# alexfreudenberg/miraculix

Measured on AMD Instinct MI355X. Metric: effective GFLOP/s for dgemm_compressed (2-bit SNP x fp64), higher is better.
Workload: dtype f64; 1 GPU; 1000000x50000 (SNPs x indiv), ncol=32, dgemm_compressed N+T per step, uncentred; snps=1000000, indiv=50000, ncol=32, parallelism=snp-shard1, form=one process per GPU

## Files before the change

miraculix_amd/csrc/mxa_kernels.hip:

```cpp
#include "mxa_internal.h"
#include "mxa_queue.h"
#include <algorithm>
#include <cstdio>
#include <cstdlib>
#include <vector>

namespace mxa {

constexpr long kMaxBlocksPerLaunch = 1L << 23;

__device__ __forceinline__ uint32_t recode16(uint32_t w) {
  const uint32_t H = (w >> 1) & 0x55555555u, L = w & 0x55555555u;
  return ((H & L) << 1) | (H & ~L);
}

__global__ void __launch_bounds__(256) k_recode(const uint8_t *__restrict__ src, size_t src_pitch, long src_row_bytes,
                                                long nrows, long k, uint8_t *__restrict__ dst, long dst_row0, long nslabs, long rows_blocks, long blk0) {
  const long bid = blk0 + blockIdx.x;
  const long rblk = bid % rows_blocks, sgrp = bid / rows_blocks;
  const int rr = threadIdx.x >> 3, part = threadIdx.x & 7;
  const long r = rblk * 32 + rr;
  const long slab = sgrp * 4 + (part >> 1);
  if (r >= nrows || slab >= nslabs) return;
  const long b = slab * kSlabBytes + (part & 1) * 16;
  uint32_t w[4] = {0u, 0u, 0u, 0u};
  const uint8_t *p = src + (size_t)r * src_pitch + b;
  if (b + 16 <= src_row_bytes && (reinterpret_cast<size_t>(p) & 3) == 0) {
    const uint32_t *q = reinterpret_cast<const uint32_t *>(p);
    w[0] = q[0]; w[1] = q[1]; w[2] = q[2]; w[3] = q[3];
  } else {
    for (int u = 0; u < 16; u++)
      if (b + u < src_row_bytes) w[u >> 2] |= (uint32_t)p[u] << (8 * (u & 3));
  }
#pragma unroll
  for (int i = 0; i < 4; i++) {
    uint32_t x = recode16(w[i]);
    const long valid = k - 4 * (b + 4 * i);
    if (valid <= 0) x = 0;
    else if (valid < 16) x &= (1u << (2 * valid)) - 1u;
    w[i] = x;
  }
  const long R = dst_row0 + r;
  const size_t off = ((size_t)(R / kTileRows) * nslabs + (size_t)slab) * kTileBytes + (size_t)(R % kTileRows) * kSlabBytes + (part & 1) * 16;
  *reinterpret_cast<uint4 *>(dst + off) = make_uint4(w[0], w[1], w[2], w[3]);
}

int launch_recode(const uint8_t *d_src, size_t src_pitch, long row0, long nrows, long k, long ,
                  PackedMatrix &dst, hipStream_t s) {
  if (nrows <= 0) return 0;
  const long rows_blocks = (nrows + 31) / 32, slab_groups = (dst.nslabs + 3) / 4;
  const long grid = rows_blocks * slab_groups;
  for (long b0 = 0; b0 < grid; b0 += kMaxBlocksPerLaunch) {
    const long nb = std::min(kMaxBlocksPerLaunch, grid - b0);
    hipLaunchKernelGGL(k_recode, dim3((unsigned)nb), dim3(256), 0, s, d_src, src_pitch, (k + 3) / 4, nrows, k, dst.d, row0, dst.nslabs, rows_blocks, b0);
  }
  MXA_HIP(hipGetLastError());
  return 0;
}

__host__ __device__ __forceinline__ long gemm_k_index(long S, int kk) { return (S >> 3) * 128 + 16 * (kk & 7) + 8 * (kk >> 3) + (S & 7); }

__global__ void __launch_bounds__(256) k_pack_B(const double *__restrict__ B, long ldb, long k, int n,
                                                double *__restrict__ Bp, long total, int C, long S_total, const int *__restrict__ E, int up, long S0, long S_cnt,
                                                const int *__restrict__ run_if_set, int rowscale) {
  if (run_if_set && *run_if_set == 0) return;
  for (long idx = (long)blockIdx.x * blockDim.x + threadIdx.x; idx < total; idx += (long)gridDim.x * blockDim.x) {
    const int l = (int)(idx & 63);
    const long sh = idx >> 6;
    const int h = (int)(sh % C);
    const long cs = sh / C;
    const long S = S0 + cs % S_cnt;
    const int chunk = (int)(cs / S_cnt);
    const long row = gemm_k_index(S, l >> 2);
    const int col = chunk * 4 * C + 4 * h + (l & 3);
    double v = 0.0;
    if (row < k && col < n) {
      v = B[row + (long)col * ldb];
      if (E) v = ldexp(v, up - E[col] - (rowscale ? 2 * (int)(row & 15) : 0));
    }
    Bp[(((size_t)chunk * S_total + S) * C + h) * 64 + l] = v;
  }
}

__global__ void __launch_bounds__(256) k_colmax_partial(const double *__restrict__ B, long ldb, long k, double *__restrict__ part, int n, int want_min) {
  const int j = blockIdx.y, c = blockIdx.x;
  const long per = (k + 63) / 64;
  const long c0 = c * per, c1 = std::min<long>(k, c0 + per);
  const double inf = __longlong_as_double(0x7ff0000000000000ll);
  double m = 0.0, lo = inf;
  for (long r = c0 + threadIdx.x; r < c1; r += 256) {
    const double a = fabs(B[r + (long)j * ldb]);
    m = (a <= 1.7976931348623157e308) ? fmax(m, a) : inf;
    if (a > 0.0) lo = fmin(lo, a);
  }
  __shared__ double sh[256], sl[256];
  sh[threadIdx.x] = m; sl[threadIdx.x] = lo;
  __syncthreads();
  for (int w = 128; w > 0; w >>= 1) {
    if ((int)threadIdx.x < w) { sh[threadIdx.x] = fmax(sh[threadIdx.x], sh[threadIdx.x + w]); sl[threadIdx.x] = fmin(sl[threadIdx.x], sl[threadIdx.x + w]); }
    __syncthreads();
  }
  if (threadIdx.x == 0) { part[(size_t)j * 64 + c] = sh[0]; if (want_min) part[((size_t)n + j) * 64 + c] = sl[0]; }
}
__global__ void k_colexp_final(const double *__restrict__ part, int n, int bias, int *__restrict__ E, int *__restrict__ flag, int max_span, int min_emax) {
  const int j = blockIdx.x * blockDim.x + threadIdx.x;
  if (j >= n) return;
  double m = 0.0;
  for (int c = 0; c < 64; c++) m = fmax(m, part[(size_t)j * 64 + c]);
  int e = 0;
  if (m > 0.0 && isfinite(m)) (void)frexp(m, &e);
  E[j] = e + bias;
  if (flag) {
    bool ok = isfinite(m);
    if (ok && m > 0.0) {
      double lo = m;
      for (int c = 0; c < 64; c++) lo = fmin(lo, part[((size_t)n + j) * 64 + c]);
      int el = 0;
      (void)frexp(lo, &el);
      ok = e >= min_emax && el >= e - max_span;
    }
    if (!ok) atomicOr(flag, 1);
  }
}
int launch_colexp(const double *dB, long ldb, long k, int n, double *d_part, int *d_E, int bias, hipStream_t s, int *d_flag, int max_span, int min_emax, bool reset_flag) {
  if (d_flag && reset_flag) MXA_HIP(hipMemsetAsync(d_flag, 0, sizeof(int), s));
  hipLaunchKernelGGL(k_colmax_partial, dim3(64, n), dim3(256), 0, s, dB, ldb, k, d_part, n, d_flag ? 1 : 0);
  hipLaunchKernelGGL(k_colexp_final, dim3((n + 63) / 64), dim3(64), 0, s, d_part, n, bias, d_E, d_flag, max_span, min_emax);
  MXA_HIP(hipGetLastError());
  return 0;
}

int launch_colexp_from_part(const double *d_part, int n, int *d_E, int bias, hipStream_t s) {
  hipLaunchKernelGGL(k_colexp_final, dim3((n + 63) / 64), dim3(64), 0, s, d_part, n, bias, d_E, (int *)nullptr, 0, 0);
  MXA_HIP(hipGetLastError());
  return 0;
}

__global__ void __launch_bounds__(256) k_colspan_final(const double *__restrict__ part, int n, int *__restrict__ out) {
  __shared__ int s_span[256], s_emax[256], s_bad[256];
  int span = 0, emin_max = 1 << 20, bad = 0;
  for (int j = threadIdx.x; j < n; j += 256) {
    double m = 0.0;
    for (int c = 0; c < 64; c++) m = fmax(m, part[(size_t)j * 64 + c]);
    if (!isfinite(m)) { bad = 1; continue; }
    if (m > 0.0) {
      double lo = m;
      for (int c = 0; c < 64; c++) lo = fmin(lo, part[((size_t)n + j) * 64 + c]);
      int e = 0, el = 0;
      (void)frexp(m, &e); (void)frexp(lo, &el);
      span = max(span, e - el); emin_max = min(emin_max, e);
    }
  }
  s_span[threadIdx.x] = span; s_emax[threadIdx.x] = emin_max; s_bad[threadIdx.x] = bad;
  __syncthreads();
  for (int w = 128; w > 0; w >>= 1) {
    if ((int)threadIdx.x < w) {
      s_span[threadIdx.x] = max(s_span[threadIdx.x], s_span[threadIdx.x + w]); s_emax[threadIdx.x] = min(s_emax[threadIdx.x], s_emax[threadIdx.x + w]);
      s_bad[threadIdx.x] |= s_bad[threadIdx.x + w];
    }
    __syncthreads();
  }
  if (threadIdx.x == 0) { out[0] = s_span[0]; out[1] = s_emax[0] == (1 << 20) ? 0 : s_emax[0]; out[2] = s_bad[0]; }
}
int launch_colspan(const double *dB, long ldb, long k, int n, double *d_part, int *d_out3, hipStream_t s) {
  hipLaunchKernelGGL(k_colmax_partial, dim3(64, n), dim3(256), 0, s, dB, ldb, k, d_part, n, 1);
  hipLaunchKernelGGL(k_colspan_final, dim3(1), dim3(256), 0, s, d_part, n, d_out3);
  MXA_HIP(hipGetLastError());
  return 0;
}

int launch_pack_B(const double *dB, long ldb, long k, int n, double *dBp, long k_pad, int n_pad, int c, hipStream_t s, const int *d_E, long S0, long S_cnt,
                  const int *run_if_set, bool rowscale) {
  const long S_total = k_pad / 16;
  if (S_cnt < 0) S_cnt = S_total - S0;
  const long total = S_cnt * (long)(n_pad / 4) * 64;
  if (total <= 0) return 0;
  const int grid = (int)std::min<long>((total + 255) / 256, 256L * 64);
  hipLaunchKernelGGL(k_pack_B, dim3(grid), dim3(256), 0, s, dB, ldb, k, n, dBp, total, c, S_total, d_E, kDenUp, S0, S_cnt, run_if_set, rowscale ? 1 : 0);
  MXA_HIP(hipGetLastError());
  return 0;
}

constexpr int kColChunks = 64;

__global__ void __launch_bounds__(256) k_colsum_partial(const double *__restrict__ B, long ldb, long k,
                                                        const double *__restrict__ f, double *__restrict__ part) {
  const int j = blockIdx.y, c = blockIdx.x;
  const long per = (k + kColChunks - 1) / kColChunks;
  const long c0 = c * per, c1 = std::min<long>(k, c0 + per);
  double s1 = 0.0, s2 = 0.0;
  for (long r = c0 + threadIdx.x; r < c1; r += 256) {
    const double b = B[r + (long)j * ldb];
    s1 += b;
    if (f) s2 = fma(f[r], b, s2);
  }
  __shared__ double sh1[256], sh2[256];
  sh1[threadIdx.x] = s1; sh2[threadIdx.x] = s2;
  __syncthreads();
  for (int w = 128; w > 0; w >>= 1) {
    if ((int)threadIdx.x < w) { sh1[threadIdx.x] += sh1[threadIdx.x + w]; sh2[threadIdx.x] += sh2[threadIdx.x + w]; }
    __syncthreads();
  }
  if (threadIdx.x == 0) {
    part[((size_t)j * kColChunks + c) * 2 + 0] = sh1[0];
    part[((size_t)j * kColChunks + c) * 2 + 1] = sh2[0];
  }
}

__global__ void k_colsum_final(const double *__restrict__ part, int n, double *__restrict__ sumB, double *__restrict__ sumfB) {
  const int j = blockIdx.x * blockDim.x + threadIdx.x;
  if (j >= n) return;
  double s1 = 0.0, s2 = 0.0;
  for (int c = 0; c < kColChunks; c++) { s1 += part[((size_t)j * kColChunks + c) * 2]; s2 += part[((size_t)j * kColChunks + c) * 2 + 1]; }
  sumB[j] = s1; sumfB[j] = s2;
}

int launch_colsums(const double *dB, long ldb, long k, int n, const double *d_f, double *d_part, double *d_sumB,
                   double *d_sumfB, hipStream_t s) {
  hipLaunchKernelGGL(k_colsum_partial, dim3(kColChunks, n), dim3(256), 0, s, dB, ldb, k, d_f, d_part);
  hipLaunchKernelGGL(k_colsum_final, dim3((n + 63) / 64), dim3(64), 0, s, d_part, n, d_sumB, d_sumfB);
  MXA_HIP(hipGetLastError());
  return 0;
}

using gptr_t = const __attribute__((address_space(1))) void *;
using lptr_t = __attribute__((address_space(3))) void *;

__device__ __forceinline__ void dma16_s(const void *sbase, uint32_t voff, uint32_t lds_addr) {
  asm volatile("s_mov_b32 m0, %2\n\ts_nop 0\n\tglobal_load_lds_dwordx4 %1, %0" ::"s"(sbase), "v"(voff), "s"(lds_addr) : "memory", "m0");
}
#ifndef MXA_NT_LUT
#define MXA_NT_LUT 0
#endif
#ifndef MXA_NT_GEMM
#define MXA_NT_GEMM 1
#endif
template <bool NT>
__device__ __forceinline__ void dma16_p(const void *sbase, uint32_t voff, uint32_t lds_addr) {
  if (NT) asm volatile("s_mov_b32 m0, %2\n\ts_nop 0\n\tglobal_load_lds_dwordx4 %1, %0 nt" ::"s"(sbase), "v"(voff), "s"(lds_addr) : "memory", "m0");
  else dma16_s(sbase, voff, lds_addr);
}

template <int A, int C>
struct GemmCfg {
  static constexpr int kRowsWave = 4 * A;
  static constexpr int kRowsWG = kWaves * kRowsWave;
  static constexpr int kBBytes = kSlabSteps * C * 512;
  static constexpr int kABytes = kRowsWG * kSlabBytes;
  static constexpr int kBufBytes = kBBytes + kABytes;
  static constexpr int kLds = 2 * kBufBytes;
  static constexpr int kBUnits = kBBytes / 1024;
  static constexpr int kAUnits = kABytes / 1024;
  static_assert(kABytes % 1024 == 0, "A tile must be a whole number of DMA units");
};

template <int A, int C, int MODE, bool DIAG = false, bool TR = false>
__global__ void __launch_bounds__(256, 2)
k_gemm(const uint8_t *__restrict__ G, size_t pitch, const double *__restrict__ Bp, int H, double *__restrict__ P,
       long m_pad, int n_pad, int rowblocks, int nchunks, int slabs_total, KSplit ks, int xcd_order,
       unsigned long long *__restrict__ diag, int split0, const int *__restrict__ run_if_set, int nunits, int *__restrict__ ctr, int g8, int p_split0) {
  using Cfg = GemmCfg<A, C>;
  extern __shared__ __attribute__((aligned(16))) char smem[];
  __shared__ int s_next;
  if (MODE == 0) { if (run_if_set && *run_if_set == 0) return; }

  const int lane = threadIdx.x & 63;
  const int wave = __builtin_amdgcn_readfirstlane(threadIdx.x >> 6);
  PieceQueue q;
  q.init(ctr, rowblocks, g8, nunits);
  auto fetch = [&]() -> int { return q.next(); };

  const uint32_t b_lane = lane * 16;
  const uint32_t a_lane = lane * 16;
  const uint32_t tr_voff = (uint32_t)((16 * ((lane >> 1) & 7) + 8 * ((lane >> 4) & 1) + (lane >> 5)) * kSlabBytes + (lane & 1) * 16);
  const size_t nslabs_all = pitch / kSlabBytes;
  const uint32_t lds0 = (uint32_t)(size_t)(lptr_t)smem;
  struct Unit { int rb, nc, sp, slab0, slab1; const char *Bp_u, *G_u; };
  auto decode = [&](int bid) -> Unit {
    Unit u;
    int grp;
    q.locate(bid, u.rb, grp);
    u.nc = grp % nchunks;
    u.sp = grp / nchunks + split0;
    u.slab0 = ksplit_begin(ks, u.sp);
    u.slab1 = u.slab0 + ksplit_len(ks, u.sp);
    const long row0 = (long)u.rb * Cfg::kRowsWG;
    u.Bp_u = reinterpret_cast<const char *>(Bp) + (size_t)u.nc * ((size_t)slabs_total * kSlabSteps * C * 512);
    if (!TR) u.G_u = reinterpret_cast<const char *>(G) + (size_t)(row0 / kTileRows) * nslabs_all * kTileBytes + (size_t)(row0 % kTileRows) * kSlabBytes;
    else u.G_u = reinterpret_cast<const char *>(G);
    return u;
  };
  auto issue = [&](const Unit &u, int slab, int buf) {
    const uint32_t base = lds0 + buf * Cfg::kBufBytes;
    const char *bslab = u.Bp_u + (size_t)slab * ((size_t)kSlabSteps * C * 512);
#pragma unroll
    for (int i = 0; i < Cfg::kBUnits / kWaves; i++) {
      const int q = wave + i * kWaves;
      dma16_s(bslab + q * 1024, b_lane, base + q * 1024);
    }
    if (!TR) {
      const char *aslab = u.G_u + (size_t)slab * kTileBytes;
#pragma unroll
      for (int i = 0; i < (Cfg::kAUnits + kWaves - 1) / kWaves; i++) {
        const int q = wave + i * kWaves;
        if (Cfg::kAUnits % kWaves == 0 || q < Cfg::kAUnits) dma16_p<MXA_NT_GEMM != 0>(aslab + q * 1024, a_lane, base + Cfg::kBBytes + q * 1024);
      }
    } else {
      constexpr int nsw = Cfg::kRowsWG / kSlabK;
      const char *arow = u.G_u + (size_t)(slab >> 1) * nslabs_all * kTileBytes + (size_t)(slab & 1) * (kTileBytes / 2);
#pragma unroll
      for (int i = 0; i < (Cfg::kAUnits + kWaves - 1) / kWaves; i++) {
        const int q = wave + i * kWaves;
        if (Cfg::kAUnits % kWaves == 0 || q < Cfg::kAUnits) {
          size_t sl = (size_t)u.rb * nsw + (q >> 2);
          if (sl >= nslabs_all) sl = nslabs_all - 1;
          dma16_p<MXA_NT_GEMM != 0>(arow + sl * kTileBytes + (q & 3) * 64, tr_voff, base + Cfg::kBBytes + q * 1024);
        }
      }
    }
  };

  typedef uint32_t u32x2 __attribute__((ext_vector_type(2)));
  u32x2 ap[A];
#pragma unroll
  for (int g = 0; g < A; g++) {
    uint32_t zero;
    asm volatile("v_mov_b32 %0, 0" : "=v"(zero));
    ap[g].x = 0; ap[g].y = zero;
  }
  uint32_t psh[kSlabSteps], pmask[kSlabSteps];
#pragma unroll
  for (int t = 0; t < kSlabSteps; t++) {
    psh[t] = 16 * (lane >> 5) + 2 * t;
    pmask[t] = 3u << psh[t];
    asm volatile("" : "+v"(pmask[t]));
  }
  const int a_off = (wave * Cfg::kRowsWave + (lane & 3)) * kSlabBytes + ((lane >> 2) & 7) * 4;
  const int b_off = lane * 8;
  const int tr_off = ((wave * A) / kSlabBytes) * (kSlabK * kSlabBytes) + (lane >> 2) * kSlabBytes + (wave * A) % kSlabBytes;
  const int tr_sh[4] = {2 * (lane & 3), 8 + 2 * (lane & 3), 16 + 2 * (lane & 3), 24 + 2 * (lane & 3)};
  const uint32_t tr_mask[4] = {3u << tr_sh[0], 3u << tr_sh[1], 3u << tr_sh[2], 3u << tr_sh[3]};
  const int j = lane & 3, blk = (lane >> 2) & 3, i = lane >> 4;

  if (threadIdx.x == 0) s_next = fetch();
  __syncthreads();
  int bid = s_next;
  if (bid < 0) return;
  Unit u = decode(bid);
  __syncthreads();
  if (u.slab0 < u.slab1) issue(u, u.slab0, 0);
  asm volatile("s_waitcnt vmcnt(0)" ::: "memory");
  __syncthreads();

  for (;;) {
    unsigned long long rt_begin = 0, t0 = 0, r0 = 0;
    if (DIAG) { rt_begin = __builtin_amdgcn_s_memrealtime(); t0 = __builtin_amdgcn_s_memtime(); r0 = rt_begin; }
    if (threadIdx.x == 0) s_next = fetch();
    if (u.slab0 >= u.slab1) __syncthreads();

    double acc[A][C];
#pragma unroll
    for (int g = 0; g < A; g++)
#pragma unroll
      for (int h = 0; h < C; h++) acc[g][h] = 0.0;

    for (int slab = u.slab0; slab < u.slab1; slab++) {
      const int buf = (slab - u.slab0) & 1;
      if (slab + 1 < u.slab1) issue(u, slab + 1, buf ^ 1);
      const char *bbase = smem + buf * Cfg::kBufBytes + b_off;
      const char *abase = smem + buf * Cfg::kBufBytes + Cfg::kBBytes + a_off;
      if (TR) {
        const char *tbase = smem + buf * Cfg::kBufBytes + Cfg::kBBytes + tr_off;
        constexpr int ND = A / 4;
        uint32_t dn[ND];
        auto load_row = [&](int kst, uint32_t (&d)[ND]) {
          if constexpr (ND == 4) { const uint4 t = *reinterpret_cast<const uint4 *>(tbase + kst * 16 * kSlabBytes); d[0] = t.x; d[1] = t.y; d[2] = t.z; d[3] = t.w; }
          else { const uint2 t = *reinterpret_cast<const uint2 *>(tbase + kst * 16 * kSlabBytes); d[0] = t.x; d[1] = t.y; }
        };
        load_row(0, dn);
#pragma unroll
        for (int kst = 0; kst < kSlabSteps; kst++) {
          uint32_t dw[ND];
#pragma unroll
          for (int t = 0; t < ND; t++) dw[t] = dn[t];
          if (kst + 1 < kSlabSteps) load_row(kst + 1, dn);
          double bf[C];
#pragma unroll
          for (int h = 0; h < C; h++) bf[h] = *reinterpret_cast<const double *>(bbase + (kst * C + h) * 512);
          double af[A];
#pragma unroll
          for (int g = 0; g < A; g++) {
            if (MODE == 3) {
              asm volatile("v_and_b32 %0, %1, %2" : "=v"(ap[g].x) : "v"(tr_mask[g & 3]), "v"(dw[g >> 2]));
              af[g] = __builtin_bit_cast(double, ap[g]);
            } else {
              const uint32_t z = __builtin_amdgcn_ubfe(dw[g >> 2], tr_sh[g & 3], 2);
              if (MODE == 0) af[g] = (double)z;
              else { ap[g].x = z; af[g] = __builtin_bit_cast(double, ap[g]); }
            }
          }
          __builtin_amdgcn_sched_barrier(0);
#pragma unroll
          for (int g = 0; g < A; g++)
#pragma unroll
            for (int h = 0; h < C; h++) acc[g][h] = __builtin_amdgcn_mfma_f64_4x4x4f64(af[g], bf[h], acc[g][h], 0, 0, 0);
          __builtin_amdgcn_sched_barrier(0);
        }
      } else {
        uint32_t aw[A];
#pragma unroll
        for (int g = 0; g < A; g++) aw[g] = *reinterpret_cast<const uint32_t *>(abase + g * 4 * kSlabBytes);
#pragma unroll
        for (int kst = 0; kst < kSlabSteps; kst++) {
          double bf[C];
#pragma unroll
          for (int h = 0; h < C; h++) bf[h] = *reinterpret_cast<const double *>(bbase + (kst * C + h) * 512);
          double af[A];
#pragma unroll
          for (int g = 0; g < A; g++) {
            if (MODE == 3) {
              asm volatile("v_and_b32 %0, %1, %2" : "=v"(ap[g].x) : "v"(pmask[kst]), "v"(aw[g]));
              af[g] = __builtin_bit_cast(double, ap[g]);
            } else {
              const uint32_t z = __builtin_amdgcn_ubfe(aw[g], psh[kst], 2);
              if (MODE == 0) af[g] = (double)z;
              else { ap[g].x = z; af[g] = __builtin_bit_cast(double, ap[g]); }
            }
          }
          __builtin_amdgcn_sched_barrier(0);
#pragma unroll
          for (int g = 0; g < A; g++)
#pragma unroll
            for (int h = 0; h < C; h++) acc[g][h] = __builtin_amdgcn_mfma_f64_4x4x4f64(af[g], bf[h], acc[g][h], 0, 0, 0);
          __builtin_amdgcn_sched_barrier(0);
        }
      }
      asm volatile("s_waitcnt vmcnt(0)" ::: "memory");
      __syncthreads();
    }

    unsigned long long t1 = 0, r1 = 0;
    if (DIAG) { t1 = __builtin_amdgcn_s_memtime(); r1 = __builtin_amdgcn_s_memrealtime(); }
    const int next = s_next;
    Unit un = u;
    if (next >= 0) { un = decode(next); if (un.slab0 < un.slab1) issue(un, un.slab0, 0); }
    constexpr int kPitch = 68;
    constexpr int kPerWave = Cfg::kBufBytes / kWaves / 8;
    constexpr int GP = (kPerWave / (C * kPitch)) < A ? (kPerWave / (C * kPitch)) : A;
    static_assert(GP >= 1, "epilogue scratch");
    double *scr = reinterpret_cast<double *>(smem + Cfg::kBufBytes) + wave * kPerWave;
    double *Pbase = P + ((size_t)(u.sp - p_split0) * rowblocks + u.rb) * ((size_t)n_pad * Cfg::kRowsWG);
#pragma unroll
    for (int g0 = 0; g0 < A; g0 += GP) {
#pragma unroll
      for (int gg = 0; gg < GP; gg++)
#pragma unroll
        for (int h = 0; h < C; h++)
          if (g0 + gg < A) scr[(gg * C + h) * kPitch + lane] = acc[g0 + gg][h];
      asm volatile("s_waitcnt lgkmcnt(0)" ::: "memory");
      __builtin_amdgcn_wave_barrier();
#pragma unroll
      for (int gg = 0; gg < GP; gg++) {
        if (g0 + gg < A) {
          const int row = wave * Cfg::kRowsWave + (g0 + gg) * 4 + i;
#pragma unroll
          for (int hq = 0; hq < C; hq += 4) {
            if (hq + blk < C) {
              const double *q = scr + (gg * C + hq + blk) * kPitch + j + 16 * i;
              double out = (q[0] + q[4]) + (q[8] + q[12]);
              if (TR && MODE == 3) out = ldexp(out, -(8 * ((g0 + gg) & 3) + 2 * i));
              const int col = 4 * (u.nc * C + hq + blk) + j;
              Pbase[(size_t)col * Cfg::kRowsWG + row] = out;
            }
          }
        }
      }
      asm volatile("s_waitcnt lgkmcnt(0)" ::: "memory");
      __builtin_amdgcn_wave_barrier();
    }
    if (DIAG && threadIdx.x == 0 && diag) {
      diag[2 * (size_t)bid] = t1 - t0; diag[2 * (size_t)bid + 1] = r1 - r0;
      diag[2 * (size_t)nunits + 2 * (size_t)bid] = rt_begin; diag[2 * (size_t)nunits + 2 * (size_t)bid + 1] = r0;
      diag[4 * (size_t)nunits + bid] = __builtin_amdgcn_s_memrealtime();
    }
    if (next < 0) break;
    u = un; bid = next;
    asm volatile("s_waitcnt vmcnt(0)" ::: "memory");
    __syncthreads();
  }
}

int gemm_default_mode(int) {
  return 3;
}

static long device_cus() {
  static const long r = [] {
    int dev = 0; hipDeviceProp_t prop;
    if (hipGetDevice(&dev) != hipSuccess || hipGetDeviceProperties(&prop, dev) != hipSuccess) { (void)hipGetLastError(); return 256L; }
    return (long)prop.multiProcessorCount;
  }();
  return r > 0 ? r : 256;
}

GemmPlan plan_gemm(long m, long k_pad, int n, const GemmPlan *ksplits_like) { return plan_gemm_host(m, k_pad, n, device_cus(), ksplits_like); }

template <int A, int C, int MODE, bool TR = false>
static int launch_gemm_t(const PackedMatrix &G, const double *dBp, double *dP, const GemmPlan &p, hipStream_t s, int split_begin, int split_end, const int *run_if_set,
                         int *d_ctr, int p_split0) {
  using Cfg = GemmCfg<A, C>;
  static unsigned long long attr_mask = 0;
  if (ensure_dyn_lds(reinterpret_cast<const void *>(&k_gemm<A, C, MODE, false, TR>), Cfg::kLds, &attr_mask)) return 1;
  const long nunits = (long)p.rowblocks * p.nchunks * (split_end - split_begin);
  if (nunits > 0x3fffffffL) { set_error(3, "launch too large"); return 1; }
  if (nunits <= 0) return 0;
  if (!d_ctr) { set_error(4, "internal: k_gemm needs its queue counters"); return 1; }
  static int per_cu[64] = {};
  int dev = 0;
  MXA_HIP(hipGetDevice(&dev));
  if (!per_cu[dev & 63]) {
    int nb = 0;
    MXA_HIP(hipOccupancyMaxActiveBlocksPerMultiprocessor(&nb, reinterpret_cast<const void *>(&k_gemm<A, C, MODE, false, TR>), 256, Cfg::kLds));
    hipDeviceProp_t prop;
    MXA_HIP(hipGetDeviceProperties(&prop, dev));
    per_cu[dev & 63] = std::max(1, std::min(nb, gemm_wg_per_cu(C))) * prop.multiProcessorCount;
  }
  const long grid = std::min<long>(nunits, per_cu[dev & 63]);
  constexpr int xcd_order = 1;
  const KSplit ks{p.s1, p.l1, p.r1, p.l2};
  const int long_groups = (std::min(split_end, p.s1) - std::min(split_begin, p.s1)) * p.nchunks;
  const int g8 = xcd_order ? (long_groups & ~7) : 0;
  MXA_HIP(hipMemsetAsync(d_ctr, 0, 9 * sizeof(int), s));
  static const bool diag_on = getenv("MXA_DIAG") != nullptr;
  if (!TR && diag_on && ((A == 8 && C == 8) || (A == 16 && C == 1)) && split_begin == 0 && split_end == p.splits && !run_if_set) {
    static unsigned long long attr2 = 0;
    if (ensure_dyn_lds(reinterpret_cast<const void *>(&k_gemm<A, C, MODE, true>), Cfg::kLds, &attr2)) return 1;
    unsigned long long *d_diag = nullptr;
    MXA_HIP(hipMalloc(reinterpret_cast<void **>(&d_diag), sizeof(unsigned long long) * 5 * nunits));
    MXA_HIP(hipMemsetAsync(d_diag, 0, sizeof(unsigned long long) * 5 * nunits, s));
    hipLaunchKernelGGL((k_gemm<A, C, MODE, true>), dim3((unsigned)grid), dim3(256), Cfg::kLds, s, G.d, G.pitch, dBp, p.n_pad / 4, dP,
                       p.m_pad, p.n_pad, p.rowblocks, p.nchunks, p.slabs_total, ks, xcd_order, d_diag, split_begin, (const int *)nullptr, (int)nunits, d_ctr, g8, p_split0);
    MXA_HIP(hipStreamSynchronize(s));
    std::vector<unsigned long long> h(5 * nunits);
    MXA_HIP(hipMemcpy(h.data(), d_diag, sizeof(unsigned long long) * 5 * nunits, hipMemcpyDeviceToHost));
    std::vector<double> ghz, cyc;
    for (long i = 0; i < nunits; i++) if (h[2 * i + 1]) {
      const int sp = (int)(i < (long)g8 * p.rowblocks ? ((i & 7) + 8 * ((i >> 3) / p.rowblocks)) / p.nchunks : (i / p.rowblocks) / p.nchunks);
      const int len = ksplit_len(ks, sp);
      ghz.push_back((double)h[2 * i] / (double)h[2 * i + 1] * 0.1); cyc.push_back((double)h[2 * i] / len);
    }
    std::sort(ghz.begin(), ghz.end()); std::sort(cyc.begin(), cyc.end());
    if (!ghz.empty()) printf("MXA_DIAG k_gemm<%d,%d,%d>: %ld pieces on %ld workgroups (splits %d = %d x %d + short x %d), in-kernel clock median %.3f GHz (min %.3f max %.3f); shader cycles per slab median %.0f (ideal %d)\n",
                             A, C, MODE, nunits, grid, p.splits, p.s1, p.l1, p.l2, ghz[ghz.size() / 2], ghz.front(), ghz.back(), cyc[cyc.size() / 2], kSlabSteps * A * C * 16 * 2);
    double ticks = 0.0;
    for (long i = 0; i < nunits; i++) ticks += (double)h[2 * i + 1];
    printf("MXA_DIAG k_gemm: K loops of all pieces = %.3f ms if packed perfectly on %ld resident slots (compare with the kernel duration)\n", ticks * 1e-5 / (double)grid, grid);
    {
      double life = 0; unsigned long long first = ~0ull, last = 0;
      for (long i = 0; i < nunits; i++) {
        const unsigned long long b = h[2 * nunits + 2 * i], e = h[4 * nunits + i];
        life += (double)(e - b);
        first = std::min(first, b); last = std::max(last, e);
      }
      printf("MXA_DIAG k_gemm: mean piece lifetime %.1f us; span first begin -> last end %.3f ms; sum of lifetimes / slots = %.3f ms\n",
             life / nunits * 1e-2, (double)(last - first) * 1e-5, life * 1e-5 / (double)grid);
      std::vector<std::pair<unsigned long long, int>> ev;
      ev.reserve(2 * nunits);
      for (long i = 0; i < nunits; i++) { ev.emplace_back(h[2 * nunits + 2 * i], +1); ev.emplace_back(h[4 * nunits + i], -1); }
      std::sort(ev.begin(), ev.end());
      const unsigned long long win = 200000;
      double idle[3] = {0, 0, 0}; long active = 0, max_active = 0; unsigned long long prev_t = first;
      for (auto &e : ev) {
        unsigned long long t0 = prev_t, t1 = e.first;
        while (t0 < t1) {
          const int zone = t0 < first + win ? 0 : (t0 >= last - win ? 2 : 1);
          const unsigned long long border = zone == 0 ? first + win : (zone == 1 ? last - win : last);
          const unsigned long long te = std::min(t1, std::max(border, t0 + 1));
          idle[zone] += (double)(te - t0) * (double)(grid - std::min(active, grid));
          t0 = te;
        }
        active += e.second; max_active = std::max(max_active, active); prev_t = e.first;
      }
      printf("MXA_DIAG k_gemm: idle slot-time first 2 ms %.3f ms, middle %.3f ms, last 2 ms %.3f ms; max pieces in flight %ld\n",
             idle[0] * 1e-5 / (double)grid, idle[1] * 1e-5 / (double)grid, idle[2] * 1e-5 / (double)grid, max_active);
    }
    (void)hipFree(d_diag);
    return 0;
  }
  hipLaunchKernelGGL((k_gemm<A, C, MODE, false, TR>), dim3((unsigned)grid), dim3(256), Cfg::kLds, s, G.d, G.pitch, dBp, p.n_pad / 4, dP,
                     p.m_pad, p.n_pad, p.rowblocks, p.nchunks, p.slabs_total, ks, xcd_order, (unsigned long long *)nullptr, split_begin, run_if_set, (int)nunits, d_ctr, g8, p_split0);
  MXA_HIP(hipGetLastError());
  return 0;
}

int launch_gemm(const PackedMatrix &G, const double *dBp, double *dP, const GemmPlan &p, int mode, hipStream_t s, int *d_ctr, int split_begin, int split_end,
                const int *run_if_set, bool tr, int p_split0) {
  if (split_end < 0) split_end = p.splits;
  if (p_split0 < 0 || p_split0 > split_begin) { set_error(4, "internal: k_gemm partial-sum base split %d outside [0, %d]", p_split0, split_begin); return 1; }
  if (!G.d) { set_error(4, "internal: k_gemm was given a packed matrix that is not stored (single-orientation object)"); return 1; }
  if (tr) {
    if ((long)p.slabs_total * kSlabK > G.rows_pad || G.nslabs < 1 || (mode != 0 && mode != 3)) {
      set_error(4, "internal: transposed launch does not fit the packed matrix (K slabs %d x 128 > %ld rows) or mode %d", p.slabs_total, G.rows_pad, mode);
      return 1;
    }
#define MXA_DISPATCH_TR(AA, CC)                                                                                          \
    if (p.a == AA && p.c == CC) {                                                                                        \
      if (mode == 3) return launch_gemm_t<AA, CC, 3, true>(G, dBp, dP, p, s, split_begin, split_end, nullptr, d_ctr, p_split0);     \
      return launch_gemm_t<AA, CC, 0, true>(G, dBp, dP, p, s, split_begin, split_end, run_if_set, d_ctr, p_split0);                 \
    }
    MXA_DISPATCH_TR(16, 1) MXA_DISPATCH_TR(16, 2) MXA_DISPATCH_TR(16, 3) MXA_DISPATCH_TR(16, 4)
    MXA_DISPATCH_TR(8, 5) MXA_DISPATCH_TR(8, 6) MXA_DISPATCH_TR(8, 7) MXA_DISPATCH_TR(8, 8)
#undef MXA_DISPATCH_TR
    set_error(5, "internal: no transposed kernel for tile a=%d c=%d", p.a, p.c);
    return 1;
  }
  if (p.m_pad > G.rows_pad || (size_t)p.slabs_total * kSlabBytes > G.pitch) {
    set_error(4, "internal: packed matrix smaller than the launch plan (m_pad %ld > %ld or k bytes %ld > pitch %zu)", p.m_pad,
              G.rows_pad, (long)p.slabs_total * kSlabBytes, G.pitch);
    return 1;
  }
#define MXA_DISPATCH(AA, CC)                                              \
  if (p.a == AA && p.c == CC) {                                           \
    if (mode == 3) return launch_gemm_t<AA, CC, 3>(G, dBp, dP, p, s, split_begin, split_end, nullptr, d_ctr, p_split0);     \
    return launch_gemm_t<AA, CC, 0>(G, dBp, dP, p, s, split_begin, split_end, run_if_set, d_ctr, p_split0);                 \
  }
  MXA_DISPATCH(16, 1)
  MXA_DISPATCH(16, 2)
  MXA_DISPATCH(16, 3)
  MXA_DISPATCH(16, 4)
  MXA_DISPATCH(8, 5)
  MXA_DISPATCH(8, 6)
  MXA_DISPATCH(8, 7)
  MXA_DISPATCH(8, 8)
#undef MXA_DISPATCH
  set_error(5, "internal: no kernel for tile a=%d c=%d", p.a, p.c);
  return 1;
}

template <int NV, int KS, int WV>
struct LutCfg {
  static constexpr int kThreads = 64 * WV;
  static constexpr int kRows = kThreads;
  static constexpr int kChunks = KS / 64;
  static constexpr int kRowBytes = kRows * KS / 4;
  static constexpr int kTabBytes = (KS / 2) * 16 * 8 * NV;
  static constexpr int kBufBytes = kRowBytes + kTabBytes;
  static constexpr int kLds = 2 * kBufBytes;
};

template <int NV, int KS, int WV>
__global__ void __launch_bounds__(64 * WV)
k_lut(const uint8_t *__restrict__ G, size_t pitch, const double *__restrict__ B, long ldb, long k, int n, double *__restrict__ P,
      long m_pad, int rowblocks, int slabs_total, int slabs_per_split, const int *__restrict__ run_if_set) {
  using Cfg = LutCfg<NV, KS, WV>;
  extern __shared__ __attribute__((aligned(16))) char smem[];
  if (run_if_set && *run_if_set == 0) return;
  const int tid = threadIdx.x, lane = tid & 63;
  const int wave = __builtin_amdgcn_readfirstlane(tid >> 6);
  const int rb = blockIdx.x % rowblocks, sp = blockIdx.x / rowblocks;
  const int slab0 = sp * slabs_per_split, slab1 = min(slab0 + slabs_per_split, slabs_total);
  const long row0 = (long)rb * Cfg::kRows;
  const uint32_t lds0 = (uint32_t)(size_t)(lptr_t)smem;
  static_assert(KS == kSlabK, "the lookup kernel walks the staged slabs");
  const uint32_t r_lane = (uint32_t)lane * kSlabBytes;
  const char *G_u = reinterpret_cast<const char *>(G) + (size_t)(row0 / kTileRows + (wave >> 2)) * (pitch / kSlabBytes) * kTileBytes +
                    (size_t)((wave & 3) * 64) * kSlabBytes;

  auto issue_rows = [&](int slab, int buf) {
    const char *src = G_u + (size_t)slab * kTileBytes;
#pragma unroll
    for (int c = 0; c < Cfg::kChunks; c++) dma16_p<MXA_NT_LUT != 0>(src + c * 16, r_lane, lds0 + buf * Cfg::kBufBytes + (c * Cfg::kRows + wave * 64) * 16);
  };
  constexpr int kEnt = (KS / 2) * 16 / Cfg::kThreads;
  static_assert((KS / 2) * 16 % Cfg::kThreads == 0, "whole entries per thread");
  auto load_b = [&](int slab, double (&b0)[kEnt][NV], double (&b1)[kEnt][NV]) {
#pragma unroll
    for (int e = 0; e < kEnt; e++) {
      const long kk = (long)slab * KS + 2 * ((tid + Cfg::kThreads * e) >> 4);
#pragma unroll
      for (int j = 0; j < NV; j++) {
        const long jc = j < n ? j : 0;
        const double v0 = B[(kk < k ? kk : k - 1) + jc * ldb];
        const double v1 = B[(kk + 1 < k ? kk + 1 : k - 1) + jc * ldb];
        b0[e][j] = (j < n && kk < k) ? v0 : 0.0;
        b1[e][j] = (j < n && kk + 1 < k) ? v1 : 0.0;
      }
    }
  };
  auto build = [&](int buf, const double (&b0)[kEnt][NV], const double (&b1)[kEnt][NV]) {
    double *tab = reinterpret_cast<double *>(smem + buf * Cfg::kBufBytes + Cfg::kRowBytes);
    const double z0 = (double)(tid & 3), z1 = (double)((tid >> 2) & 3);
#pragma unroll
    for (int e = 0; e < kEnt; e++)
#pragma unroll
      for (int j = 0; j < NV; j++) tab[(size_t)(tid + Cfg::kThreads * e) * NV + j] = fma(z1, b1[e][j], z0 * b0[e][j]);
  };

  double acc[4][NV];
#pragma unroll
  for (int a = 0; a < 4; a++)
#pragma unroll
    for (int j = 0; j < NV; j++) acc[a][j] = 0.0;

  double bc0[kEnt][NV], bc1[kEnt][NV], bn0[kEnt][NV], bn1[kEnt][NV];
  if (slab0 < slab1) {
    issue_rows(slab0, 0);
    load_b(slab0, bc0, bc1);
    build(0, bc0, bc1);
    if (slab0 + 1 < slab1) load_b(slab0 + 1, bc0, bc1);
  }
  asm volatile("s_waitcnt vmcnt(0)" ::: "memory");
  __syncthreads();
  for (int slab = slab0; slab < slab1; slab++) {
    const int buf = (slab - slab0) & 1;
    if (slab + 1 < slab1) {
      issue_rows(slab + 1, buf ^ 1);
      if (slab + 2 < slab1) load_b(slab + 2, bn0, bn1);
      build(buf ^ 1, bc0, bc1);
#pragma unroll
      for (int e = 0; e < kEnt; e++)
#pragma unroll
        for (int j = 0; j < NV; j++) { bc0[e][j] = bn0[e][j]; bc1[e][j] = bn1[e][j]; }
    }
    const char *rows = smem + buf * Cfg::kBufBytes + tid * 16;
    const uint32_t tab = lds0 + buf * Cfg::kBufBytes + Cfg::kRowBytes;
#pragma unroll
    for (int c = 0; c < Cfg::kChunks; c++) {
      const uint4 w4 = *reinterpret_cast<const uint4 *>(rows + c * Cfg::kRows * 16);
#pragma unroll
      for (int d = 0; d < 4; d++) {
        const uint32_t w = d == 0 ? w4.x : d == 1 ? w4.y : d == 2 ? w4.z : w4.w;
#pragma unroll
        for (int q = 0; q < 8; q++) {
          const uint32_t idx = __builtin_amdgcn_ubfe(w, 4 * q, 4);
          uint32_t addr;
          if (NV == 1) asm("v_lshl_or_b32 %0, %1, 3, %2" : "=v"(addr) : "v"(idx), "v"(tab));
          else if (NV == 2) asm("v_lshl_or_b32 %0, %1, 4, %2" : "=v"(addr) : "v"(idx), "v"(tab));
          else asm("v_lshl_or_b32 %0, %1, 5, %2" : "=v"(addr) : "v"(idx), "v"(tab));
          __builtin_assume((addr & (8 * NV - 1)) == 0);
          using lds_cd = const __attribute__((address_space(3))) double;
          lds_cd *e = (lds_cd *)(size_t)(addr + (c * 32 + d * 8 + q) * 16 * 8 * NV);
#pragma unroll
          for (int j = 0; j < NV; j++) acc[q & 3][j] += e[j];
        }
      }
    }
    asm volatile("s_waitcnt vmcnt(0)" ::: "memory");
    __syncthreads();
  }
  double *Pbase = P + (size_t)sp * NV * m_pad;
#pragma unroll
  for (int j = 0; j < NV; j++) Pbase[(size_t)j * m_pad + row0 + tid] = (acc[0][j] + acc[1][j]) + (acc[2][j] + acc[3][j]);
}

constexpr int kLutWaves = 8;

template <int NV, int KS>
static int launch_lut_t(const PackedMatrix &G, const double *dB, long ldb, int n, double *dP, const GemmPlan &p, hipStream_t s, const int *run_if_set) {
  using Cfg = LutCfg<NV, KS, kLutWaves>;
  static unsigned long long attr_mask = 0;
  if (ensure_dyn_lds(reinterpret_cast<const void *>(&k_lut<NV, KS, kLutWaves>), Cfg::kLds, &attr_mask)) return 1;
  const long grid = (long)p.rowblocks * p.splits;
  hipLaunchKernelGGL((k_lut<NV, KS, kLutWaves>), dim3((unsigned)grid), dim3(Cfg::kThreads), Cfg::kLds, s, G.d, G.pitch, dB, ldb, G.k, n, dP, p.m_pad,
                     p.rowblocks, p.slabs_total, p.slabs_per_split, run_if_set);
  MXA_HIP(hipGetLastError());
  return 0;
}

constexpr int kLutKS = 128;

GemmPlan plan_lut(long m, long k_pad, int n) { return plan_lut_host(m, k_pad, n); }

static_assert(kPlanWaves == kWaves && kPlanSlabSteps == kSlabSteps && kPlanSlabK == kSlabK && kPlanLutWaves == kLutWaves && kPlanLutKS == kLutKS,
              "mxa_plan.h restates the kernels' geometry for the host-only planners");

int launch_lut(const PackedMatrix &G, const double *dB, long ldb, int n, double *dP, const GemmPlan &p, hipStream_t s, const int *run_if_set) {
  if (!G.d) { set_error(4, "internal: k_lut was given a packed matrix that is not stored (single-orientation object)"); return 1; }
  if (p.m_pad > G.rows_pad || (size_t)p.slabs_total * (kLutKS / 4) > G.pitch) { set_error(4, "internal: packed matrix smaller than the lookup plan"); return 1; }
  if (p.n_pad == 1) return launch_lut_t<1, kLutKS>(G, dB, ldb, n, dP, p, s, run_if_set);
  if (p.n_pad == 2) return launch_lut_t<2, kLutKS>(G, dB, ldb, n, dP, p, s, run_if_set);
  return launch_lut_t<4, kLutKS>(G, dB, ldb, n, dP, p, s, run_if_set);
}

__global__ void __launch_bounds__(256) k_finish(const double *__restrict__ P, long m_pad, long p_rows, int p_shift, int n_pad, int splits, long m, int n,
                                                double *__restrict__ Cout, long ldc, long fill_rows, int mode_trans, int centered,
                                                const double *__restrict__ sumB, const double *__restrict__ sumfB,
                                                const double *__restrict__ f, const int *__restrict__ E, int back, int e_splits, int e_stride,
                                                const int *__restrict__ run_if_set, const int *__restrict__ unscaled_if_set, int group) {
  const int j = blockIdx.y;
  const long r0 = 2 * ((long)blockIdx.x * blockDim.x + threadIdx.x);
  if (run_if_set && *run_if_set == 0) return;
  if (unscaled_if_set && *unscaled_if_set != 0) E = nullptr;
  if (r0 >= fill_rows) return;
  const bool acc_in = group & 1, raw_out = group & 2;
  const bool two = r0 + 1 < fill_rows;
  double *cp = Cout + r0 + (long)j * ldc;
  double v0 = 0.0, v1 = 0.0;
  if (acc_in) { if (r0 < m) v0 = cp[0]; if (two && r0 + 1 < m) v1 = cp[1]; }
  if (r0 < m) {
    const size_t tile = p_shift >= 0 ? (size_t)(r0 >> p_shift) : (size_t)(r0 / p_rows), within = p_shift >= 0 ? (size_t)(r0 & (p_rows - 1)) : (size_t)(r0 % p_rows);
    const size_t ntiles = p_shift >= 0 ? (size_t)(m_pad >> p_shift) : (size_t)(m_pad / p_rows);
    const size_t sstride = ntiles * (size_t)n_pad * (size_t)p_rows;
    const double *pp = P + ((tile * n_pad + j) * (size_t)p_rows + within);
    typedef double v2d __attribute__((ext_vector_type(2)));
    const bool per_split_scale = !raw_out && E && e_splits > 0;
    for (int s = 0; s < splits; s++) {
      const v2d x = __builtin_nontemporal_load(reinterpret_cast<const v2d *>(pp + (size_t)s * sstride));
      if (per_split_scale) {
        const int ex = back + E[(size_t)(s / e_splits) * e_stride + j];
        v0 += ldexp(x[0], ex); v1 += ldexp(x[1], ex);
      } else { v0 += x[0]; v1 += x[1]; }
    }
    if (!raw_out) {
      if (E && !per_split_scale) { const int ex = back + E[j]; v0 = ldexp(v0, ex); v1 = ldexp(v1, ex); }
      if (centered) {
        if (mode_trans) { const double c = -2.0 * sumB[j]; v0 = fma(c, f[r0], v0); if (r0 + 1 < m) v1 = fma(c, f[r0 + 1], v1); }
        else { const double c = -2.0 * sumfB[j]; v0 += c; v1 += c; }
      }
    }
    if (r0 + 1 >= m) v1 = 0.0;
  }
  if (two && (reinterpret_cast<size_t>(cp) & 15) == 0) {
    typedef double v2d __attribute__((ext_vector_type(2)));
    *reinterpret_cast<v2d *>(cp) = v2d{v0, v1};
  } else { cp[0] = v0; if (two) cp[1] = v1; }
}

int launch_finish(const double *dP, const GemmPlan &p, long m, int n, double *dC, long ldc, long fill_rows, int mode_trans, bool centered,
                  const double *d_sumB, const double *d_sumfB, const double *d_f, hipStream_t s, const int *d_E, int e_splits, int e_stride, const int *run_if_set,
                  const int *unscaled_if_set, int group_splits, int group) {
  if ((p.p_rows & 1) || (p.m_pad & 1)) { set_error(4, "internal: k_finish wants even tile heights (p_rows %ld, m_pad %ld)", p.p_rows, p.m_pad); return 1; }
  int p_shift = -1;
  if ((p.p_rows & (p.p_rows - 1)) == 0) { p_shift = 0; while ((1L << p_shift) < p.p_rows) p_shift++; }
  dim3 grid((unsigned)((fill_rows + 511) / 512), n);
  hipLaunchKernelGGL(k_finish, grid, dim3(256), 0, s, dP, p.m_pad, p.p_rows, p_shift, p.n_pad, group_splits > 0 ? group_splits : p.splits, m, n, dC, ldc, fill_rows, mode_trans,
                     centered ? 1 : 0, d_sumB, d_sumfB, d_f, d_E, 1074 - kDenUp, e_splits, e_stride, run_if_set, unscaled_if_set, group);
  MXA_HIP(hipGetLastError());
  return 0;
}


__global__ void __launch_bounds__(256) k_reduce_parts(PartList parts, long m, double *__restrict__ Cout, long ldc, long fill_rows) {
  const int j = blockIdx.y;
  const long r = (long)blockIdx.x * blockDim.x + threadIdx.x;
  if (r >= fill_rows) return;
  double v = 0.0;
  if (r < m) {
    v = parts.p[0][r + (size_t)j * m];
    for (int g = 1; g < parts.count; g++) v += parts.p[g][r + (size_t)j * m];
  }
  Cout[r + (size_t)j * ldc] = v;
}

int launch_reduce_parts(const PartList &parts, long m, int n, double *dC, long ldc, long fill_rows, hipStream_t s) {
  if (n <= 0 || parts.count <= 0) return 0;
  dim3 grid((unsigned)((fill_rows + 255) / 256), n);
  hipLaunchKernelGGL(k_reduce_parts, grid, dim3(256), 0, s, parts, m, dC, ldc, fill_rows);
  MXA_HIP(hipGetLastError());
  return 0;
}

int ensure_dyn_lds(const void *func, int bytes, unsigned long long *mask) {
  int dev = 0;
  MXA_HIP(hipGetDevice(&dev));
  const unsigned long long bit = 1ull << (dev & 63);
  if (__atomic_load_n(mask, __ATOMIC_ACQUIRE) & bit) return 0;
  MXA_HIP(hipFuncSetAttribute(func, hipFuncAttributeMaxDynamicSharedMemorySize, bytes));
  __atomic_fetch_or(mask, bit, __ATOMIC_RELEASE);
  return 0;
}

template <bool ALIGNED>
__global__ void __launch_bounds__(256) k_transpose_2bit(const uint8_t *__restrict__ in, long rows, long cols,
                                                        uint8_t *__restrict__ out, long nbx, long blk0) {
  __shared__ uint8_t tile[64][20];
  const long bin = (cols + 3) / 4, bout = (rows + 3) / 4;
  const long bid = blk0 + blockIdx.x;
  const long r0 = (bid / nbx) * 64, c0 = (bid % nbx) * 64;
  {
    const int r = threadIdx.x >> 2, part = threadIdx.x & 3;
    const long byte0 = c0 / 4 + part * 4;
    uint32_t w = 0;
    if (r0 + r < rows) {
      if (ALIGNED && byte0 + 3 < bin) {
        w = *reinterpret_cast<const uint32_t *>(in + (size_t)(r0 + r) * bin + byte0);
      } else {
        for (int u = 0; u < 4; u++)
          if (byte0 + u < bin) w |= (uint32_t)in[(size_t)(r0 + r) * bin + byte0 + u] << (8 * u);
      }
    }
    *reinterpret_cast<uint32_t *>(&tile[r][part * 4]) = w;
  }
  __syncthreads();
  {
    const int c = threadIdx.x >> 2, q = threadIdx.x & 3;
    if (c0 + c < cols) {
      const long obyte0 = r0 / 4 + 4 * q;
      uint32_t wout = 0;
      for (int ob = 0; ob < 4; ob++) {
        uint32_t v = 0;
        for (int u = 0; u < 4; u++) {
          const int r = 16 * q + 4 * ob + u;
          uint32_t code = (tile[r][c >> 2] >> (2 * (c & 3))) & 3u;
          if (r0 + r >= rows) code = 0;
          v |= code << (2 * u);
        }
        wout |= v << (8 * ob);
      }
      if (ALIGNED && obyte0 + 3 < bout) {
        *reinterpret_cast<uint32_t *>(out + (size_t)(c0 + c) * bout + obyte0) = wout;
      } else {
        for (int ob = 0; ob < 4; ob++)
          if (obyte0 + ob < bout) out[(size_t)(c0 + c) * bout + obyte0 + ob] = (uint8_t)(wout >> (8 * ob));
      }
    }
  }
}

__device__ __forceinline__ void swap_fields(uint32_t &lo, uint32_t &hi, int sh, uint32_t mask) {
  const uint32_t t = ((lo >> sh) ^ hi) & mask;
  hi ^= t;
  lo ^= t << sh;
}
__device__ __forceinline__ void transpose16x16_2bit(uint32_t (&a)[16]) {
#pragma unroll
  for (int i = 0; i < 8; i++) swap_fields(a[i], a[i + 8], 16, 0x0000FFFFu);
#pragma unroll
  for (int i = 0; i < 16; i++) if (!(i & 4)) swap_fields(a[i], a[i + 4], 8, 0x00FF00FFu);
#pragma unroll
  for (int i = 0; i < 16; i++) if (!(i & 2)) swap_fields(a[i], a[i + 2], 4, 0x0F0F0F0Fu);
#pragma unroll
  for (int i = 0; i < 16; i++) if (!(i & 1)) swap_fields(a[i], a[i + 1], 2, 0x33333333u);
}

struct __attribute__((packed, aligned(4))) U4 { uint32_t x[4]; };
constexpr int kTrRows = 256, kTrCols = 512;
constexpr int kTrInPitch = kTrCols / 16 + 1;
constexpr int kTrOutPitch = kTrRows / 16 + 1;

__global__ void __launch_bounds__(256) k_transpose_2bit_tiled(const uint8_t *__restrict__ in, long rows, long cols, uint8_t *__restrict__ out, long nbx, long blk0) {
  __shared__ uint32_t lds[(kTrRows * kTrInPitch > kTrCols * kTrOutPitch) ? kTrRows * kTrInPitch : kTrCols * kTrOutPitch];
  const long bin = (cols + 3) / 4, bout = (rows + 3) / 4;
  const long bid = blk0 + blockIdx.x;
  const long r0 = (bid / nbx) * kTrRows, c0 = (bid % nbx) * kTrCols;
  const long din = bin / 4, dout = bout / 4;
  const uint32_t *in32 = reinterpret_cast<const uint32_t *>(in);
  uint32_t *out32 = reinterpret_cast<uint32_t *>(out);
#pragma unroll
  for (int it = 0; it < 8; it++) {
    const int idx = threadIdx.x + 256 * it;
    const int r = idx >> 3, part = idx & 7;
    const long gr = r0 + r, gd = c0 / 16 + part * 4;
    uint32_t w[4] = {0u, 0u, 0u, 0u};
    if (gr < rows) {
      const uint32_t *p = in32 + (size_t)gr * din + gd;
      if (gd + 3 < din) { const U4 v = *reinterpret_cast<const U4 *>(p); w[0] = v.x[0]; w[1] = v.x[1]; w[2] = v.x[2]; w[3] = v.x[3]; }
      else { for (int u = 0; u < 4; u++) if (gd + u < din) w[u] = p[u]; }
    }
#pragma unroll
    for (int u = 0; u < 4; u++) lds[r * kTrInPitch + part * 4 + u] = w[u];
  }
  __syncthreads();
  uint32_t a[2][16];
#pragma unroll
  for (int pass = 0; pass < 2; pass++) {
    const int bc = threadIdx.x & 31, br = (threadIdx.x >> 5) + 8 * pass;
#pragma unroll
    for (int i = 0; i < 16; i++) a[pass][i] = lds[(16 * br + i) * kTrInPitch + bc];
    transpose16x16_2bit(a[pass]);
  }
  __syncthreads();
#pragma unroll
  for (int pass = 0; pass < 2; pass++) {
    const int bc = threadIdx.x & 31, br = (threadIdx.x >> 5) + 8 * pass;
#pragma unroll
    for (int f = 0; f < 16; f++) lds[(16 * bc + f) * kTrOutPitch + br] = a[pass][f];
  }
  __syncthreads();
#pragma unroll
  for (int it = 0; it < 8; it++) {
    const int idx = threadIdx.x + 256 * it;
    const int orow = idx >> 2, part = idx & 3;
    const long gc = c0 + orow, gd = r0 / 16 + part * 4;
    if (gc < cols) {
      uint32_t *p = out32 + (size_t)gc * dout + gd;
      U4 v;
#pragma unroll
      for (int u = 0; u < 4; u++) v.x[u] = lds[orow * kTrOutPitch + part * 4 + u];
      if (gd + 3 < dout) *reinterpret_cast<U4 *>(p) = v;
      else { for (int u = 0; u < 4; u++) if (gd + u < dout) p[u] = v.x[u]; }
    }
  }
}

int launch_transpose_2bit(const uint8_t *d_in, long rows, long cols, uint8_t *d_out, hipStream_t s) {
  if (rows <= 0 || cols <= 0) return 0;
  const long bin = (cols + 3) / 4, bout = (rows + 3) / 4;
  const bool aligned = (bin % 4 == 0) && (bout % 4 == 0) && (reinterpret_cast<uintptr_t>(d_in) % 4 == 0) && (reinterpret_cast<uintptr_t>(d_out) % 4 == 0);
  constexpr bool no_tiled = false;
  if (aligned && !no_tiled) {
    const long nbx = (cols + kTrCols - 1) / kTrCols, nby = (rows + kTrRows - 1) / kTrRows;
    for (long b0 = 0; b0 < nbx * nby; b0 += kMaxBlocksPerLaunch)
      hipLaunchKernelGGL(k_transpose_2bit_tiled, dim3((unsigned)std::min(kMaxBlocksPerLaunch, nbx * nby - b0)), dim3(256), 0, s, d_in, rows, cols, d_out, nbx, b0);
    MXA_HIP(hipGetLastError());
    return 0;
  }
  const long nbx = (cols + 63) / 64, nby = (rows + 63) / 64;
  for (long b0 = 0; b0 < nbx * nby; b0 += kMaxBlocksPerLaunch) {
    const unsigned nb = (unsigned)std::min(kMaxBlocksPerLaunch, nbx * nby - b0);
    if (aligned) hipLaunchKernelGGL(k_transpose_2bit<true>, dim3(nb), dim3(256), 0, s, d_in, rows, cols, d_out, nbx, b0);
    else hipLaunchKernelGGL(k_transpose_2bit<false>, dim3(nb), dim3(256), 0, s, d_in, rows, cols, d_out, nbx, b0);
  }
  MXA_HIP(hipGetLastError());
  return 0;
}

__device__ __forceinline__ unsigned count16(uint32_t w) {
  const uint32_t z = recode16(w);
  const uint32_t s2 = (z & 0x33333333u) + ((z >> 2) & 0x33333333u);
  const uint32_t s4 = (s2 & 0x0F0F0F0Fu) + ((s2 >> 4) & 0x0F0F0F0Fu);
  return (s4 * 0x01010101u) >> 24;
}

__global__ void __launch_bounds__(256) k_allele_freq(const uint8_t *__restrict__ plink, long snps, long indiv, double *__restrict__ f) {
  const long s = (long)blockIdx.x * 4 + (threadIdx.x >> 6);
  const int lane = threadIdx.x & 63;
  if (s >= snps) return;
  const long bps = (indiv + 3) / 4;
  const uint8_t *row = plink + (size_t)s * bps;
  unsigned long long cnt = 0;
  const long full = indiv / 4;
  long head = (long)((16 - (reinterpret_cast<uintptr_t>(row) & 15)) & 15);
  if (head > full) head = full;
  const long nvec = (full - head) / 16;
  for (long v = lane; v < nvec; v += 64) {
    const uint4 w = *reinterpret_cast<const uint4 *>(row + head + v * 16);
    cnt += count16(w.x) + count16(w.y) + count16(w.z) + count16(w.w);
  }
  for (long b = lane; b < head; b += 64) cnt += count16(row[b]);
  for (long b = head + nvec * 16 + lane; b < bps; b += 64) {
    uint32_t w = row[b];
    long valid = indiv - 4 * b;
    if (valid < 4) w &= (1u << (2 * valid)) - 1u;
    cnt += count16(w);
  }
  for (int o = 32; o > 0; o >>= 1) cnt += __shfl_xor(cnt, o);
  if (lane == 0) f[s] = (double)cnt / (2.0 * (double)indiv);
}

int launch_allele_freq(const uint8_t *d_plink, long snps, long indiv, double *d_f, hipStream_t s) {
  if (snps <= 0) return 0;
  hipLaunchKernelGGL(k_allele_freq, dim3((unsigned)((snps + 3) / 4)), dim3(256), 0, s, d_plink, snps, indiv, d_f);
  MXA_HIP(hipGetLastError());
  return 0;
}

}
```

Before: 74490 GFLOP/s.

## Stage B packing through LDS tile for coalesced reads and vectorized writes

Rewrites k_pack_B so that each block handles one slab of rows for one column chunk. A wave reads contiguous rows of each B column, so loads are coalesced, and the block scatters the values into a padded shared-memory fragment. It then writes the packed layout out with 2-wide vector stores. The old grid-stride loop did gather-style strided reads per element. The new kernel assumes c<=8, adds validation for that, and uses one block per slab-chunk.

```diff
diff --git a/miraculix_amd/csrc/mxa_kernels.hip b/miraculix_amd/csrc/mxa_kernels.hip
--- a/miraculix_amd/csrc/mxa_kernels.hip
+++ b/miraculix_amd/csrc/mxa_kernels.hip
@@ -60,25 +60,64 @@
 
 __host__ __device__ __forceinline__ long gemm_k_index(long S, int kk) { return (S >> 3) * 128 + 16 * (kk & 7) + 8 * (kk >> 3) + (S & 7); }
 
+constexpr int kPackFragPitch = 65;
 __global__ void __launch_bounds__(256) k_pack_B(const double *__restrict__ B, long ldb, long k, int n,
                                                 double *__restrict__ Bp, long total, int C, long S_total, const int *__restrict__ E, int up, long S0, long S_cnt,
                                                 const int *__restrict__ run_if_set, int rowscale) {
+  (void)total;
   if (run_if_set && *run_if_set == 0) return;
-  for (long idx = (long)blockIdx.x * blockDim.x + threadIdx.x; idx < total; idx += (long)gridDim.x * blockDim.x) {
-    const int l = (int)(idx & 63);
-    const long sh = idx >> 6;
-    const int h = (int)(sh % C);
-    const long cs = sh / C;
-    const long S = S0 + cs % S_cnt;
-    const int chunk = (int)(cs / S_cnt);
-    const long row = gemm_k_index(S, l >> 2);
-    const int col = chunk * 4 * C + 4 * h + (l & 3);
-    double v = 0.0;
-    if (row < k && col < n) {
-      v = B[row + (long)col * ldb];
-      if (E) v = ldexp(v, up - E[col] - (rowscale ? 2 * (int)(row & 15) : 0));
-    }
-    Bp[(((size_t)chunk * S_total + S) * C + h) * 64 + l] = v;
+  __shared__ double frag[kSlabSteps * 8 * kPackFragPitch];
+  const long sl0 = S0 / kSlabSteps, nsl = (S0 + S_cnt + kSlabSteps - 1) / kSlabSteps - sl0;
+  const int chunk = (int)(blockIdx.x / nsl);
+  const long sl = sl0 + (long)blockIdx.x % nsl;
+  const int lane = threadIdx.x & 63, wave = threadIdx.x >> 6;
+  double v[2 * 8];
+  long cc[8];
+#pragma unroll
+  for (int i = 0; i < 8; i++) {
+    const int cl = wave + 4 * i < 4 * C ? wave + 4 * i : 4 * C - 1;
+    const int col = chunk * 4 * C + cl;
+    cc[i] = col < n ? col : n - 1;
+#pragma unroll
+    for (int hf = 0; hf < 2; hf++) {
+      const long row = sl * kSlabK + lane + 64 * hf;
+      v[2 * i + hf] = B[(row < k ? row : k - 1) + cc[i] * ldb];
+    }
+  }
+  int ev[8];
+  if (E) {
+#pragma unroll
+    for (int i = 0; i < 8; i++) ev[i] = up - E[cc[i]];
+  } else {
+#pragma unroll
+    for (int i = 0; i < 8; i++) ev[i] = 0;
+  }
+#pragma unroll
+  for (int i = 0; i < 8; i++) {
+    if (wave + 4 * i >= 4 * C) break;
+    const int cl = wave + 4 * i, col = chunk * 4 * C + cl;
+#pragma unroll
+    for (int hf = 0; hf < 2; hf++) {
+      const int r = lane + 64 * hf;
+      const long row = sl * kSlabK + r;
+      double x = 0.0;
+      if (row < k && col < n) {
+        x = v[2 * i + hf];
+        if (E) x = ldexp(x, ev[i] - (rowscale ? 2 * (int)(row & 15) : 0));
+      }
+      const int t = r & 7, kk = (r >> 4) + 8 * ((r >> 3) & 1);
+      frag[(t * C + (cl >> 2)) * kPackFragPitch + 4 * kk + (cl & 3)] = x;
+    }
+  }
+  __syncthreads();
+  double *dst = Bp + ((size_t)chunk * S_total + (size_t)sl * kSlabSteps) * C * 64;
+  const int pairs = kSlabSteps * C * 32;
+  for (int p = threadIdx.x; p < pairs; p += 256) {
+    const int th = p >> 5, l = 2 * (p & 31);
+    const long S = sl * kSlabSteps + th / C;
+    if (S < S0 || S >= S0 + S_cnt) continue;
+    typedef double v2d __attribute__((ext_vector_type(2)));
+    *reinterpret_cast<v2d *>(dst + (size_t)th * 64 + l) = v2d{frag[th * kPackFragPitch + l], frag[th * kPackFragPitch + l + 1]};
   }
 }
 
@@ -175,8 +214,10 @@
   if (S_cnt < 0) S_cnt = S_total - S0;
   const long total = S_cnt * (long)(n_pad / 4) * 64;
   if (total <= 0) return 0;
-  const int grid = (int)std::min<long>((total + 255) / 256, 256L * 64);
-  hipLaunchKernelGGL(k_pack_B, dim3(grid), dim3(256), 0, s, dB, ldb, k, n, dBp, total, c, S_total, d_E, kDenUp, S0, S_cnt, run_if_set, rowscale ? 1 : 0);
+  if (c < 1 || c > 8 || n_pad % (4 * c) != 0 || k < 1 || n < 1) { set_error(4, "internal: k_pack_B tile c = %d, n_pad = %d, k = %ld, n = %d", c, n_pad, k, n); return 1; }
+  const long nsl = (S0 + S_cnt + kSlabSteps - 1) / kSlabSteps - S0 / kSlabSteps, grid = nsl * (n_pad / (4 * c));
+  if (grid > 0x7fffffffL) { set_error(3, "k_pack_B: launch too large"); return 1; }
+  hipLaunchKernelGGL(k_pack_B, dim3((unsigned)grid), dim3(256), 0, s, dB, ldb, k, n, dBp, total, c, S_total, d_E, kDenUp, S0, S_cnt, run_if_set, rowscale ? 1 : 0);
   MXA_HIP(hipGetLastError());
   return 0;
 }
```

After: 74580 GFLOP/s, median of 6. No clear change (+0.1%).
